# TongtongSong/OpenEAT

Measured on AMD Instinct MI355X. Metric: audio-frames/sec/GPU (train) + RTF (attention-rescoring decode), 12L Conformer, higher is better.
Workload: dtype f32 (storage, accumulate, softmax, norms, losses, optimizer all fp32; every matrix product is the fp32 product to within one fp32 rounding, computed as six exact bf16 x bf16 MFMA products of three-piece operand splits h+m+l = x, dropped terms < 2^-24 |a||b| - tests hold it to the exact-fp32 mode's t; 1 GPU; configs[1]: 12L Conformer d=256 (12+3+3, h=4, ff=1024, K=15, V=3246), B=32/GPU x 10 s 16 kHz wav (T=998 frames), L=30, CTC+attention joint loss, fbank+fwd+bwd+clip+Adam, dropout 0.1; global_batch=32, parallelism=dp1, hip_graph=True

## Files before the change

openeat_amd/csrc/conv.hip:

```cpp
#include <stdlib.h>
#include "oe_common.h"
#include "../../include/openeat_hip.h"

__global__ __launch_bounds__(256) void conv1_fwd_kernel(const float* __restrict__ x, const float* __restrict__ w,
                                                         const float* __restrict__ bias, int B, int T, int F, int T1, int F1,
                                                         int C, int pos_per_block, float* __restrict__ y,
                                                         __bf16* __restrict__ y_planes, long plane_stride) {
    const int cpt = C >> 2;
    const int grp = threadIdx.x / cpt;
    const int c4 = (threadIdx.x % cpt) * 4;
    const int ngrp = blockDim.x / cpt;
    float wr[4][9], br[4];
#pragma unroll
    for (int e = 0; e < 4; ++e) {
        br[e] = bias[c4 + e];
#pragma unroll
        for (int k = 0; k < 9; ++k) wr[e][k] = w[(c4 + e) * 9 + k];
    }
    const long npos = (long)B * T1 * F1;
    const long p0 = (long)blockIdx.x * pos_per_block;
    for (long pos = p0 + grp; pos < min(npos, p0 + pos_per_block); pos += ngrp) {
        const int f = (int)(pos % F1);
        const int t = (int)((pos / F1) % T1);
        const long b = pos / ((long)F1 * T1);
        const float* xp = x + (b * T + 2 * t) * F + 2 * f;
        float xv[9];
#pragma unroll
        for (int kh = 0; kh < 3; ++kh)
#pragma unroll
            for (int kw = 0; kw < 3; ++kw) xv[kh * 3 + kw] = xp[kh * F + kw];
        float o[4];
#pragma unroll
        for (int e = 0; e < 4; ++e) {
            float s = br[e];
#pragma unroll
            for (int k = 0; k < 9; ++k) s += wr[e][k] * xv[k];
            o[e] = fmaxf(s, 0.f);
        }
        const float4 o4 = make_float4(o[0], o[1], o[2], o[3]);
        if (y) *reinterpret_cast<float4*>(y + pos * C + c4) = o4;
        if (y_planes) store_planes4(y_planes + pos * C + c4, plane_stride, o4);
    }
}

template <int UB, bool UNIFORM>
__global__ __launch_bounds__(UNIFORM ? 512 : 256) void conv1_wgrad_kernel(const float* __restrict__ x, const float* __restrict__ dy, int B, int T,
                                                           int F, int T1, int F1, int C, int pos_per_block,
                                                           float* __restrict__ dw, float* __restrict__ db) {
    const int cpt = C >> 2;
    const int grp = UNIFORM ? __builtin_amdgcn_readfirstlane(threadIdx.x >> 6) : threadIdx.x / cpt;
    const int c4 = (threadIdx.x % cpt) * 4;
    const int ngrp = blockDim.x / cpt;
    float acc[4][10];
#pragma unroll
    for (int e = 0; e < 4; ++e)
#pragma unroll
        for (int k = 0; k < 10; ++k) acc[e][k] = 0.f;
    const long npos = (long)B * T1 * F1;
    const long p0 = (long)blockIdx.x * pos_per_block;
    const long pstart = p0 + grp, pend = min(npos, p0 + pos_per_block);
    int f = (int)(pstart % F1), t = (int)((pstart / F1) % T1);
    long b = pstart / ((long)F1 * T1);
    for (long pos = pstart; pos < pend; pos += (long)UB * ngrp) {
        float xv[UB][9];
        float4 g4[UB];
#pragma unroll
        for (int u = 0; u < UB; ++u) {
            const long pu = pos + (long)u * ngrp;
            const bool ok = pu < pend;
            const float* xp = x + (b * T + 2 * t) * F + 2 * f;
#pragma unroll
            for (int kh = 0; kh < 3; ++kh)
#pragma unroll
                for (int kw = 0; kw < 3; ++kw) xv[u][kh * 3 + kw] = ok ? xp[kh * F + kw] : 0.f;
            g4[u] = ok ? *reinterpret_cast<const float4*>(dy + pu * C + c4) : make_float4(0.f, 0.f, 0.f, 0.f);
            f += ngrp;
            while (f >= F1) { f -= F1; if (++t == T1) { t = 0; ++b; } }
            if (b >= B) { b = B - 1; t = 0; f = 0; }
        }
#pragma unroll
        for (int u = 0; u < UB; ++u) {
            const float g[4] = {g4[u].x, g4[u].y, g4[u].z, g4[u].w};
#pragma unroll
            for (int e = 0; e < 4; ++e) {
#pragma unroll
                for (int k = 0; k < 9; ++k) acc[e][k] += g[e] * xv[u][k];
                acc[e][9] += g[e];
            }
        }
    }
    extern __shared__ float sh[];
    if (UNIFORM) {
        for (int i = threadIdx.x; i < C * 10; i += blockDim.x) sh[i] = 0.f;
        __syncthreads();
#pragma unroll
        for (int e = 0; e < 4; ++e)
#pragma unroll
            for (int k = 0; k < 10; ++k) atomicAdd(&sh[(c4 + e) * 10 + k], acc[e][k]);
        __syncthreads();
        for (int i = threadIdx.x; i < C * 10; i += blockDim.x) {
            const int c = i / 10, k = i % 10;
            if (k < 9) atomicAdd(dw + c * 9 + k, sh[i]); else atomicAdd(db + c, sh[i]);
        }
        return;
    }
#pragma unroll
    for (int e = 0; e < 4; ++e)
#pragma unroll
        for (int k = 0; k < 10; ++k) sh[(grp * C + c4 + e) * 10 + k] = acc[e][k];
    __syncthreads();
    for (int i = threadIdx.x; i < C * 10; i += blockDim.x) {
        float s = 0.f;
        for (int gq = 0; gq < ngrp; ++gq) s += sh[gq * C * 10 + i];
        const int c = i / 10, k = i % 10;
        if (k < 9) atomicAdd(dw + c * 9 + k, s); else atomicAdd(db + c, s);
    }
}

static int conv1_block(int C) {
    const int cpt = C / 4;
    return cpt * (256 / cpt > 0 ? 256 / cpt : 1);
}

extern "C" int oe_conv1_fwd_pl(const float* x, const float* w, const float* bias, int B, int T, int F, int C, float* y,
                               void* y_planes, long plane_stride, void* stream);
extern "C" int oe_conv1_fwd(const float* x, const float* w, const float* bias, int B, int T, int F, int C, float* y,
                            void* stream) {
    return oe_conv1_fwd_pl(x, w, bias, B, T, F, C, y, nullptr, 0, stream);
}
extern "C" int oe_conv1_fwd_pl(const float* x, const float* w, const float* bias, int B, int T, int F, int C, float* y,
                               void* y_planes, long plane_stride, void* stream) {
    OE_REQUIRE(x && w && bias && (y || y_planes), "oe_conv1_fwd: null pointer");
    OE_REQUIRE(!y_planes || ((((uintptr_t)y_planes) & 7) == 0 && plane_stride % 4 == 0), "oe_conv1_fwd_pl: planes must be 8-byte aligned");
    OE_REQUIRE(B > 0 && T >= 3 && F >= 3 && C > 0 && C % 4 == 0 && C <= 1024, "oe_conv1_fwd: bad shape (C %% 4 == 0, C <= 1024)");
    const int T1 = (T - 3) / 2 + 1, F1 = (F - 3) / 2 + 1;
    const long npos = (long)B * T1 * F1;
    const int ppb = 64;
    hipLaunchKernelGGL(conv1_fwd_kernel, dim3(oe_cdiv(npos, ppb)), dim3(conv1_block(C)), 0, (hipStream_t)stream, x, w, bias, B, T,
                       F, T1, F1, C, ppb, y, (__bf16*)y_planes, plane_stride);
    OE_LAUNCH_CHECK("conv1_fwd");
    return 0;
}

extern "C" int oe_conv1_wgrad(const float* x, const float* dy, int B, int T, int F, int C, float* dw, float* db, void* stream) {
    OE_REQUIRE(x && dy && dw && db, "oe_conv1_wgrad: null pointer");
    OE_REQUIRE(B > 0 && T >= 3 && F >= 3 && C > 0 && C % 4 == 0 && C <= 1024, "oe_conv1_wgrad: bad shape");
    const int T1 = (T - 3) / 2 + 1, F1 = (F - 3) / 2 + 1;
    const long npos = (long)B * T1 * F1;
    static const int ppb_env = getenv("OE_CONV1_WGRAD_PPB") ? atoi(getenv("OE_CONV1_WGRAD_PPB")) : 0;
    static const int variant = getenv("OE_CONV1_WGRAD") ? atoi(getenv("OE_CONV1_WGRAD")) : 0;
    const bool uni = (C == 256) && variant != 1;
    const int ppb = ppb_env > 0 ? ppb_env : (uni ? (int)max(256L, (npos + 511) / 512) : 512);
    const int threads = uni ? 512 : conv1_block(C);
    const int ngrp = threads / (C / 4);
    const size_t lds = uni ? (size_t)C * 10 * sizeof(float) : (size_t)ngrp * C * 10 * sizeof(float);
#define C1W(UBB, UNI) hipLaunchKernelGGL((conv1_wgrad_kernel<UBB, UNI>), dim3(oe_cdiv(npos, ppb)), dim3(threads), lds, (hipStream_t)stream, x, dy, B, T, F, T1,  \
                                         F1, C, ppb, dw, db)
    if (uni && variant == 8) C1W(8, true);
    else if (uni) C1W(4, true);
    else if (variant == 1) C1W(1, false);
    else C1W(4, false);
#undef C1W
    OE_LAUNCH_CHECK("conv1_wgrad");
    return 0;
}

__global__ __launch_bounds__(256) void col2im_relu_kernel(const float* __restrict__ dcol, const float* __restrict__ y1, int B,
                                                           int T1, int F1, int T2, int F2, int C, int KS, int S,
                                                           float* __restrict__ dx) {
    const long idx = (long)blockIdx.x * blockDim.x + threadIdx.x;
    const int cv = C >> 2;
    const long total = (long)B * T1 * F1 * cv;
    if (idx >= total) return;
    const int c = (int)(idx % cv) * 4;
    const long pos = idx / cv;
    const int f1 = (int)(pos % F1);
    const int t1 = (int)((pos / F1) % T1);
    const long b = pos / ((long)F1 * T1);
    float4 s = make_float4(0.f, 0.f, 0.f, 0.f);
    for (int kh = 0; kh < KS; ++kh) {
        const int tt = t1 - kh;
        if (tt < 0 || (tt % S) || (tt / S) >= T2) continue;
        for (int kw = 0; kw < KS; ++kw) {
            const int ff = f1 - kw;
            if (ff < 0 || (ff % S) || (ff / S) >= F2) continue;
            const long m = (b * T2 + (tt / S)) * F2 + (ff / S);
            const float4 v = *reinterpret_cast<const float4*>(dcol + m * ((long)KS * KS * C) + (kh * KS + kw) * C + c);
            s.x += v.x; s.y += v.y; s.z += v.z; s.w += v.w;
        }
    }
    const float4 y = *reinterpret_cast<const float4*>(y1 + pos * C + c);
    s.x = y.x > 0.f ? s.x : 0.f; s.y = y.y > 0.f ? s.y : 0.f; s.z = y.z > 0.f ? s.z : 0.f; s.w = y.w > 0.f ? s.w : 0.f;
    *reinterpret_cast<float4*>(dx + pos * C + c) = s;
}

extern "C" int oe_col2im_relu_ks(const float* dcol, const float* y1, int B, int T1, int F1, int C, int KS, int S, float* dx,
                                 void* stream) {
    OE_REQUIRE(dcol && y1 && dx && B > 0 && KS >= 1 && S >= 1 && T1 >= KS && F1 >= KS && C > 0 && C % 4 == 0, "oe_col2im_relu: bad arguments");
    const int T2 = (T1 - KS) / S + 1, F2 = (F1 - KS) / S + 1;
    const long total = (long)B * T1 * F1 * (C / 4);
    hipLaunchKernelGGL(col2im_relu_kernel, dim3(oe_cdiv(total, 256)), dim3(256), 0, (hipStream_t)stream, dcol, y1, B, T1, F1, T2,
                       F2, C, KS, S, dx);
    OE_LAUNCH_CHECK("col2im_relu");
    return 0;
}
extern "C" int oe_col2im_relu(const float* dcol, const float* y1, int B, int T1, int F1, int C, float* dx, void* stream) {
    return oe_col2im_relu_ks(dcol, y1, B, T1, F1, C, 3, 2, dx, stream);
}

#ifdef OE_GEMM_STAMPS
static __device__ unsigned long long* oe_dw_stamp_buf = nullptr;
extern "C" int oe_debug_set_dw_stamp_buffer(void* p) { return (int)hipMemcpyToSymbol(HIP_SYMBOL(oe_dw_stamp_buf), &p, sizeof(p)); }
#define DW_STAMP(slot)                                                                                         \
    do {                                                                                                       \
        __builtin_amdgcn_sched_barrier(0);                                                                     \
        unsigned long long t_;                                                                                 \
        asm volatile("s_memtime %0\n\ts_waitcnt lgkmcnt(0)" : "=s"(t_) :: "memory");                           \
        __builtin_amdgcn_sched_barrier(0);                                                                     \
        if (oe_dw_stamp_buf && threadIdx.x == 0 && blockIdx.y < 8) oe_dw_stamp_buf[(blockIdx.y * 16 + (blockIdx.x & 15)) * 8 + (slot)] = t_; \
    } while (0)
#else
#define DW_STAMP(slot) do { } while (0)
#endif

#define DW_TT 16
#define DW_MAXK 31
template <int KT, bool EXACT>
__global__ __launch_bounds__(256) void dwconv_glu_fwd_kernel(const float* __restrict__ a, const float* __restrict__ w,
                                                              const float* __restrict__ bias, const float* __restrict__ gpad,
                                                              int T, int d, int K, int pad_left, float* __restrict__ y,
                                                              const float* __restrict__ ln_gamma, const float* __restrict__ ln_beta, float ln_eps,
                                                              int ln_act, float* __restrict__ z, float* __restrict__ ln_stats) {
    extern __shared__ __attribute__((aligned(16))) float win[];
    const int b = blockIdx.y;
    const int t0 = blockIdx.x * DW_TT;
    const int rows = DW_TT + K - 1;
    const int dv = d >> 2;
    for (int e0 = threadIdx.x; e0 < rows * dv; e0 += 256 * 4) {
        float4 xv[4], gv[4];
        int kind[4];
#pragma unroll
        for (int u = 0; u < 4; ++u) {
            const int e = e0 + u * 256;
            kind[u] = 0;
            xv[u] = gv[u] = make_float4(0.f, 0.f, 0.f, 0.f);
            if (e < rows * dv) {
                const int r = e / dv, c = (e % dv) * 4;
                const int t = t0 - pad_left + r;
                if (t >= 0 && t < T) {
                    const float* ap = a + ((long)b * T + t) * 2 * d;
                    xv[u] = *reinterpret_cast<const float4*>(ap + c);
                    gv[u] = *reinterpret_cast<const float4*>(ap + d + c);
                    kind[u] = 1;
                } else if (t < 0 && gpad) {
                    xv[u] = *reinterpret_cast<const float4*>(gpad + c);
                    kind[u] = 2;
                }
            }
        }
#pragma unroll
        for (int u = 0; u < 4; ++u) {
            const int e = e0 + u * 256;
            if (e < rows * dv) {
                const int r = e / dv, c = (e % dv) * 4;
                float4 g = xv[u];
                if (kind[u] == 1)
                    g = make_float4(xv[u].x * sigmoidf_(gv[u].x), xv[u].y * sigmoidf_(gv[u].y), xv[u].z * sigmoidf_(gv[u].z), xv[u].w * sigmoidf_(gv[u].w));
                *reinterpret_cast<float4*>(win + r * d + c) = g;
            }
        }
    }
    __syncthreads();
    for (int c = threadIdx.x; c < d; c += 256) {
        float wk[KT];
#pragma unroll
        for (int k = 0; k < KT; ++k) wk[k] = (EXACT || k < K) ? w[c * K + k] : 0.f;
        const float bc = bias[c];
#pragma unroll
        for (int tt = 0; tt < DW_TT; ++tt) {
            const int t = t0 + tt;
            float s = bc;
#pragma unroll
            for (int k = 0; k < KT; ++k) if (EXACT || k < K) s += wk[k] * win[(tt + k) * d + c];
            if (t < T) y[((long)b * T + t) * d + c] = s;
            if (z) win[(rows + tt) * d + c] = s;
        }
    }
    if (z == nullptr) return;
    __syncthreads();
    const int lane = threadIdx.x & 63, wave = threadIdx.x >> 6;
    const float4* g4 = reinterpret_cast<const float4*>(ln_gamma);
    const float4* b4 = reinterpret_cast<const float4*>(ln_beta);
    for (int tt = wave; tt < DW_TT; tt += 4) {
        const int t = t0 + tt;
        if (t >= T) break;
        const float4* yr = reinterpret_cast<const float4*>(win + (rows + tt) * d);
        float sum = 0.f;
        for (int i = lane; i < dv; i += 64) { const float4 v = yr[i]; sum += v.x + v.y + v.z + v.w; }
        const float mean = wave_sum(sum) / d;
        float q = 0.f;
        for (int i = lane; i < dv; i += 64) {
            const float4 v = yr[i];
            const float p0 = v.x - mean, p1 = v.y - mean, p2 = v.z - mean, p3 = v.w - mean;
            q += p0 * p0 + p1 * p1 + p2 * p2 + p3 * p3;
        }
        const float rstd = rsqrtf(wave_sum(q) / d + ln_eps);
        const long row = (long)b * T + t;
        if (lane == 0) { ln_stats[row * 2] = mean; ln_stats[row * 2 + 1] = rstd; }
        float4* zr = reinterpret_cast<float4*>(z + row * d);
        for (int i = lane; i < dv; i += 64) {
            const float4 v = yr[i], g = g4[i], bb = b4[i];
            zr[i] = make_float4(act_fwd(ln_act, (v.x - mean) * rstd * g.x + bb.x), act_fwd(ln_act, (v.y - mean) * rstd * g.y + bb.y),
                                act_fwd(ln_act, (v.z - mean) * rstd * g.z + bb.z), act_fwd(ln_act, (v.w - mean) * rstd * g.w + bb.w));
        }
    }
}

template <int KT, bool EXACT>
__global__ __launch_bounds__(256) void dwconv_glu_bwd_kernel(const float* __restrict__ a, const float* __restrict__ dy,
                                                              const float* __restrict__ w, const float* __restrict__ gpad,
                                                              int T, int d, int K, int pad_left,
                                                              float* __restrict__ da, float* __restrict__ partial,
                                                              float* __restrict__ dgpad) {
    extern __shared__ __attribute__((aligned(16))) float sh[];
    const int rows = DW_TT + K - 1;
    float* gwin = sh;
    float* dwin = sh + rows * d;
    const int b = blockIdx.y;
    const int t0 = blockIdx.x * DW_TT;
    const int dv = d >> 2;
    DW_STAMP(0);
    for (int e0 = threadIdx.x; e0 < rows * dv; e0 += 256 * 8) {
        float4 xv[8], gv[8], qv[8];
        int kind[8];
#pragma unroll
        for (int u = 0; u < 8; ++u) {
            const int e = e0 + u * 256;
            kind[u] = 0;
            xv[u] = gv[u] = qv[u] = make_float4(0.f, 0.f, 0.f, 0.f);
            if (e < rows * dv) {
                const int r = e / dv, c = (e % dv) * 4;
                const int tg = t0 - pad_left + r;
                if (tg >= 0 && tg < T) {
                    const float* ap = a + ((long)b * T + tg) * 2 * d;
                    xv[u] = *reinterpret_cast<const float4*>(ap + c);
                    gv[u] = *reinterpret_cast<const float4*>(ap + d + c);
                    kind[u] = 1;
                } else if (tg < 0 && gpad) {
                    xv[u] = *reinterpret_cast<const float4*>(gpad + c);
                    kind[u] = 2;
                }
                const int td = t0 + pad_left - (K - 1) + r;
                if (td >= 0 && td < T) qv[u] = *reinterpret_cast<const float4*>(dy + ((long)b * T + td) * d + c);
            }
        }
#pragma unroll
        for (int u = 0; u < 8; ++u) {
            const int e = e0 + u * 256;
            if (e < rows * dv) {
                const int r = e / dv, c = (e % dv) * 4;
                float4 g = xv[u];
                if (kind[u] == 1)
                    g = make_float4(xv[u].x * sigmoidf_(gv[u].x), xv[u].y * sigmoidf_(gv[u].y), xv[u].z * sigmoidf_(gv[u].z), xv[u].w * sigmoidf_(gv[u].w));
                *reinterpret_cast<float4*>(gwin + r * d + c) = g;
                *reinterpret_cast<float4*>(dwin + r * d + c) = qv[u];
            }
        }
    }
    DW_STAMP(1);
    __syncthreads();
    DW_STAMP(2);
    for (int c = threadIdx.x; c < d; c += 256) {
        float wk[KT], dwk[KT];
#pragma unroll
        for (int k = 0; k < KT; ++k) { wk[k] = (EXACT || k < K) ? w[c * K + k] : 0.f; dwk[k] = 0.f; }
        float dbs = 0.f;
        float xs[DW_TT], gs[DW_TT];
#pragma unroll
        for (int tt = 0; tt < DW_TT; ++tt) {
            const int t = min(t0 + tt, T - 1);
            const float* ap = a + ((long)b * T + t) * 2 * d;
            xs[tt] = ap[c];
            gs[tt] = ap[d + c];
        }
        DW_STAMP(3);
#pragma unroll
        for (int tt = 0; tt < DW_TT; ++tt) {
            const int t = t0 + tt;
            if (t < T) {
            float dg = 0.f;
#pragma unroll
            for (int k = 0; k < KT; ++k) if (EXACT || k < K) dg += wk[k] * dwin[(tt + (K - 1) - k) * d + c];
            const float xv = xs[tt], gv = gs[tt];
            const float sg = sigmoidf_(gv);
            float* dap = da + ((long)b * T + t) * 2 * d;
            dap[c] = dg * sg;
            dap[d + c] = dg * xv * sg * (1.f - sg);
            const float dyt = dwin[(tt + (K - 1) - pad_left) * d + c];
            dbs += dyt;
#pragma unroll
            for (int k = 0; k < KT; ++k) if (EXACT || k < K) dwk[k] += dyt * gwin[(tt + k) * d + c];
            }
        }
        DW_STAMP(4);
        float* pp = partial + ((long)(blockIdx.y * gridDim.x + blockIdx.x) * (K + 1)) * d + c;
#pragma unroll
        for (int k = 0; k < KT; ++k) if (EXACT || k < K) pp[(long)k * d] = dwk[k];
        pp[(long)K * d] = dbs;
        DW_STAMP(5);
        if (dgpad && blockIdx.x == 0) {
            float acc = 0.f;
            const int td0 = pad_left - (K - 1);
            for (int tau = -pad_left; tau < 0; ++tau)
#pragma unroll
                for (int k = 0; k < KT; ++k) {
                    const int td = tau + pad_left - k;
                    if ((EXACT || k < K) && td >= 0 && td - td0 < rows) acc += wk[k] * dwin[(td - td0) * d + c];
                }
            atomicAdd(dgpad + c, acc);
        }
    }
}

#define DW_PR_ROWS 64
__global__ __launch_bounds__(256) void dwconv_param_reduce_kernel(const float* __restrict__ partial, int nblocks, int d, int K,
                                                                   float* __restrict__ dw, float* __restrict__ db) {
    __shared__ float sh[4][64];
    const int cx = threadIdx.x & 63, ry = threadIdx.x >> 6;
    const int idx = blockIdx.x * 64 + cx;
    const int n = (K + 1) * d;
    const int b0 = blockIdx.y * DW_PR_ROWS, b1 = min(nblocks, b0 + DW_PR_ROWS);
    float s = 0.f;
    if (idx < n) {
#pragma unroll 4
        for (int b = b0 + ry; b < b1; b += 4) s += partial[(long)b * n + idx];
    }
    sh[ry][cx] = s;
    __syncthreads();
    if (ry == 0 && idx < n) {
        const float v = sh[0][cx] + sh[1][cx] + sh[2][cx] + sh[3][cx];
        const int k = idx / d, c = idx % d;
        if (k < K) atomicAdd(dw + c * K + k, v); else atomicAdd(db + c, v);
    }
}

extern "C" size_t oe_dwconv_glu_bwd_workspace_floats(int B, int T, int d, int K) {
    return (size_t)B * oe_cdiv(T, DW_TT) * (K + 1) * d;
}

extern "C" int oe_dwconv_glu_ln_fwd(const float* a, const float* w, const float* bias, const float* gpad, int B, int T, int d,
                                    int K, int causal, float* y, const float* ln_gamma, const float* ln_beta, float ln_eps, int ln_act,
                                    float* z, float* ln_stats, void* stream);
extern "C" int oe_dwconv_glu_fwd(const float* a, const float* w, const float* bias, const float* gpad, int B, int T, int d,
                                 int K, int causal, float* y, void* stream) {
    return oe_dwconv_glu_ln_fwd(a, w, bias, gpad, B, T, d, K, causal, y, nullptr, nullptr, 0.f, 0, nullptr, nullptr, stream);
}
extern "C" int oe_dwconv_glu_ln_fwd(const float* a, const float* w, const float* bias, const float* gpad, int B, int T, int d,
                                    int K, int causal, float* y, const float* ln_gamma, const float* ln_beta, float ln_eps, int ln_act,
                                    float* z, float* ln_stats, void* stream) {
    OE_REQUIRE(a && w && bias && y, "oe_dwconv_glu_fwd: null pointer");
    OE_REQUIRE(!z || (ln_gamma && ln_beta && ln_stats), "oe_dwconv_glu_ln_fwd: the fused LayerNorm needs gamma, beta and a statistics buffer");
    OE_REQUIRE(B > 0 && T > 0 && d > 0 && d % 4 == 0 && K >= 1 && K <= DW_MAXK, "oe_dwconv_glu_fwd: bad shape (d %% 4, K <= %d)", DW_MAXK);
    OE_REQUIRE(causal || (K % 2 == 1), "oe_dwconv_glu_fwd: kernel size must be odd for the symmetric convolution");
    const int pad_left = causal ? K - 1 : (K - 1) / 2;
    const size_t lds = (size_t)(DW_TT + K - 1 + (z ? DW_TT : 0)) * d * sizeof(float);
    OE_REQUIRE(lds <= 160 * 1024, "oe_dwconv_glu_fwd: window does not fit LDS (d=%d)", d);
#define DW_FWD(KT, EX)                                                                                                           \
    do {                                                                                                                     \
        if (lds > 48 * 1024) (void)hipFuncSetAttribute((const void*)dwconv_glu_fwd_kernel<KT, EX>, hipFuncAttributeMaxDynamicSharedMemorySize, (int)lds); \
        hipLaunchKernelGGL((dwconv_glu_fwd_kernel<KT, EX>), dim3(oe_cdiv(T, DW_TT), B), dim3(256), lds, (hipStream_t)stream, a, w, bias, gpad, T, d, \
                           K, pad_left, y, ln_gamma, ln_beta, ln_eps, ln_act, z, ln_stats);                                  \
    } while (0)
    if (K == 15) DW_FWD(15, true); else if (K == 7) DW_FWD(7, true); else if (K == 31) DW_FWD(31, true);
    else if (K < 7) DW_FWD(7, false); else if (K < 15) DW_FWD(15, false); else DW_FWD(31, false);
#undef DW_FWD
    OE_LAUNCH_CHECK("dwconv_glu_fwd");
    return 0;
}

extern "C" int oe_dwconv_glu_bwd(const float* a, const float* dy, const float* w, const float* gpad, int B, int T, int d, int K,
                                 int causal, float* da, float* dw, float* db, float* dgpad, float* workspace, void* stream) {
    OE_REQUIRE(a && dy && w && da && dw && db && workspace, "oe_dwconv_glu_bwd: null pointer");
    OE_REQUIRE(!dgpad || (K - 1 <= DW_TT + K - 1), "oe_dwconv_glu_bwd: pad window");
    OE_REQUIRE(B > 0 && T > 0 && d > 0 && d % 4 == 0 && K >= 1 && K <= DW_MAXK, "oe_dwconv_glu_bwd: bad shape");
    const int pad_left = causal ? K - 1 : (K - 1) / 2;
    const size_t lds = (size_t)2 * (DW_TT + K - 1) * d * sizeof(float);
    OE_REQUIRE(lds <= 160 * 1024, "oe_dwconv_glu_bwd: window does not fit LDS (d=%d)", d);
#define DW_BWD(KT, EX)                                                                                                           \
    do {                                                                                                                     \
        if (lds > 48 * 1024) (void)hipFuncSetAttribute((const void*)dwconv_glu_bwd_kernel<KT, EX>, hipFuncAttributeMaxDynamicSharedMemorySize, (int)lds); \
        hipLaunchKernelGGL((dwconv_glu_bwd_kernel<KT, EX>), dim3(oe_cdiv(T, DW_TT), B), dim3(256), lds, (hipStream_t)stream, a, dy, w, gpad, T, d, \
                           K, pad_left, da, workspace, dgpad);                                                               \
    } while (0)
    if (K == 15) DW_BWD(15, true); else if (K == 7) DW_BWD(7, true); else if (K == 31) DW_BWD(31, true);
    else if (K < 7) DW_BWD(7, false); else if (K < 15) DW_BWD(15, false); else DW_BWD(31, false);
#undef DW_BWD
    OE_LAUNCH_CHECK("dwconv_glu_bwd");
    hipLaunchKernelGGL(dwconv_param_reduce_kernel, dim3(oe_cdiv((K + 1) * d, 64), oe_cdiv(B * oe_cdiv(T, DW_TT), DW_PR_ROWS)), dim3(256), 0, (hipStream_t)stream, workspace,
                       B * oe_cdiv(T, DW_TT), d, K, dw, db);
    OE_LAUNCH_CHECK("dwconv_param_reduce");
    return 0;
}


__global__ __launch_bounds__(256) void pad1_nhwc_kernel(const float4* __restrict__ dy, int B, int To, int Fo, int C4, float4* __restrict__ out) {
    const long n = (long)B * (To + 2) * (Fo + 2) * C4;
    for (long i = (long)blockIdx.x * 256 + threadIdx.x; i < n; i += (long)gridDim.x * 256) {
        const int c = (int)(i % C4);
        long q = i / C4;
        const int f = (int)(q % (Fo + 2)) - 1;
        q /= (Fo + 2);
        const int t = (int)(q % (To + 2)) - 1;
        const long b = q / (To + 2);
        float4 v = make_float4(0.f, 0.f, 0.f, 0.f);
        if (t >= 0 && t < To && f >= 0 && f < Fo) v = dy[((b * To + t) * Fo + f) * C4 + c];
        out[i] = v;
    }
}
extern "C" int oe_pad1_nhwc(const float* dy, int B, int To, int Fo, int C, float* out, void* stream) {
    OE_REQUIRE(dy && out && B > 0 && To > 0 && Fo > 0 && C > 0 && C % 4 == 0, "oe_pad1_nhwc: bad arguments (C must be a multiple of 4)");
    OE_REQUIRE((((uintptr_t)dy | (uintptr_t)out) & 15) == 0, "oe_pad1_nhwc: pointers must be 16-byte aligned");
    const long n = (long)B * (To + 2) * (Fo + 2) * (C / 4);
    hipLaunchKernelGGL(pad1_nhwc_kernel, dim3((unsigned)min((long)oe_cdiv(n, 256), 65536L)), dim3(256), 0, (hipStream_t)stream,
                       (const float4*)dy, B, To, Fo, C / 4, (float4*)out);
    OE_LAUNCH_CHECK("pad1_nhwc");
    return 0;
}
__global__ __launch_bounds__(256) void pad1_nhwc_planes_kernel(const float4* __restrict__ dy, int B, int To, int Fo, int C4, float4* __restrict__ out,
                                                                __bf16* __restrict__ planes, long pstride) {
    const long n = (long)B * (To + 2) * (Fo + 2) * C4;
    for (long i = (long)blockIdx.x * 256 + threadIdx.x; i < n; i += (long)gridDim.x * 256) {
        const int c = (int)(i % C4);
        long q = i / C4;
        const int f = (int)(q % (Fo + 2)) - 1;
        q /= (Fo + 2);
        const int t = (int)(q % (To + 2)) - 1;
        const long b = q / (To + 2);
        float4 v = make_float4(0.f, 0.f, 0.f, 0.f);
        if (t >= 0 && t < To && f >= 0 && f < Fo) v = dy[((b * To + t) * Fo + f) * C4 + c];
        if (out) out[i] = v;
        store_planes4(planes + 4 * i, pstride, v);
    }
}
extern "C" int oe_pad1_nhwc_planes(const float* dy, int B, int To, int Fo, int C, float* out, void* planes, long plane_stride, void* stream) {
    OE_REQUIRE(dy && planes && B > 0 && To > 0 && Fo > 0 && C > 0 && C % 4 == 0, "oe_pad1_nhwc_planes: bad arguments (C must be a multiple of 4)");
    OE_REQUIRE((((uintptr_t)dy | (uintptr_t)out) & 15) == 0 && (((uintptr_t)planes) & 7) == 0 && plane_stride % 4 == 0,
               "oe_pad1_nhwc_planes: dy / out must be 16-byte, the planes 8-byte aligned");
    const long n = (long)B * (To + 2) * (Fo + 2) * (C / 4);
    hipLaunchKernelGGL(pad1_nhwc_planes_kernel, dim3((unsigned)min((long)oe_cdiv(n, 256), 65536L)), dim3(256), 0, (hipStream_t)stream,
                       (const float4*)dy, B, To, Fo, C / 4, (float4*)out, (__bf16*)planes, plane_stride);
    OE_LAUNCH_CHECK("pad1_nhwc_planes");
    return 0;
}
__global__ __launch_bounds__(256) void conv_dgrad_k3s2_weights_kernel(const float* __restrict__ w, int C, float* __restrict__ out) {
    const long n = 9L * C * C;
    const long i = (long)blockIdx.x * 256 + threadIdx.x;
    if (i >= n) return;
    const long cc = (long)C * C;
    int cls, KH, KW;
    long base;
    if (i < 4 * cc) { cls = 0; KH = 2; KW = 2; base = 0; }
    else if (i < 6 * cc) { cls = 1; KH = 2; KW = 1; base = 4 * cc; }
    else if (i < 8 * cc) { cls = 2; KH = 1; KW = 2; base = 6 * cc; }
    else { cls = 3; KH = 1; KW = 1; base = 8 * cc; }
    const long r = i - base;
    const int co = (int)(r % C);
    long q = r / C;
    const int kwi = (int)(q % KW);
    q /= KW;
    const int khi = (int)(q % KH);
    const int ci = (int)(q / KH);
    const int kh = (cls >> 1) ? 1 : (khi == 0 ? 2 : 0);
    const int kw = (cls & 1) ? 1 : (kwi == 0 ? 2 : 0);
    out[i] = w[(((long)co * C + ci) * 3 + kh) * 3 + kw];
}
extern "C" int oe_conv_dgrad_k3s2_weights(const float* w, int C, float* out, void* stream) {
    OE_REQUIRE(w && out && C > 0, "oe_conv_dgrad_k3s2_weights: bad arguments");
    hipLaunchKernelGGL(conv_dgrad_k3s2_weights_kernel, dim3(oe_cdiv(9L * C * C, 256)), dim3(256), 0, (hipStream_t)stream, w, C, out);
    OE_LAUNCH_CHECK("conv_dgrad_k3s2_weights");
    return 0;
}
```

openeat_amd/csrc/fbank.hip:

```cpp
#include "oe_common.h"
#include "../../include/openeat_hip.h"

#define FB_WAVES 4
#define FB_MAX_NFFT 1024

#define FB_WAVE_SYNC()                                            \
    do {                                                          \
        asm volatile("s_waitcnt lgkmcnt(0)" ::: "memory");        \
        __builtin_amdgcn_wave_barrier();                          \
    } while (0)
template <int FB_NFFT>
__global__ __launch_bounds__(64 * FB_WAVES) void fbank_kernel(const float* __restrict__ wav, const int* __restrict__ nsamples,
                                                              int B, long wav_stride, int Tmax, int win, int hop, int n_mel,
                                                              float scale, float preemph, const float* __restrict__ window,
                                                              const float* __restrict__ twiddle, const int* __restrict__ mel_start,
                                                              const int* __restrict__ mel_off, const float* __restrict__ mel_w,
                                                              float floor_eps, const float* __restrict__ cmvn_mean,
                                                              const float* __restrict__ cmvn_istd, float* __restrict__ out,
                                                              float dither, unsigned long long dither_seed) {
    __shared__ float2 bufA[FB_WAVES][FB_NFFT];
    __shared__ float2 bufB[FB_WAVES][FB_NFFT];
    __shared__ float2 tw[FB_NFFT / 2];
    for (int i = threadIdx.x; i < FB_NFFT / 2; i += 64 * FB_WAVES) tw[i] = reinterpret_cast<const float2*>(twiddle)[i];
    __syncthreads();
    const int lane = threadIdx.x & 63, wave = threadIdx.x >> 6;
    const long frame = (long)blockIdx.x * FB_WAVES + wave;
    const bool live_frame = frame < (long)B * Tmax;
    const int b = live_frame ? (int)(frame / Tmax) : 0;
    const int t = live_frame ? (int)(frame % Tmax) : 0;
    const int ns = nsamples ? nsamples[b] : (int)wav_stride;
    const int Tb = ns < win ? 0 : 1 + (ns - win) / hop;
    const bool live = live_frame && t < Tb;
    float2* A = bufA[wave];
    float2* Bf = bufB[wave];
    float part = 0.f;
    const float* src = wav + (long)b * wav_stride + (long)t * hop;
    for (int i = lane; i < FB_NFFT; i += 64) {
        float v = 0.f;
        if (live && i < win) {
            v = src[i] * scale;
            if (dither != 0.f) {
                const uint4 h = philox4(dither_seed, (unsigned long long)frame * FB_NFFT + i);
                const float u1 = ((float)(h.x >> 8) + 0.5f) * (1.f / 16777216.f), u2 = (float)(h.y >> 8) * (1.f / 16777216.f);
                v += dither * sqrtf(-2.f * __logf(u1)) * __cosf(6.283185307179586f * u2);
            }
        }
        A[i].x = v;
        part += v;
    }
    const float mean = wave_sum(part) / (float)win;
    FB_WAVE_SYNC();
    for (int i = lane; i < FB_NFFT; i += 64) {
        float v = 0.f;
        if (i < win) {
            const float cur = A[i].x - mean;
            const float prev = A[i > 0 ? i - 1 : 0].x - mean;
            v = (cur - preemph * prev) * window[i];
        }
        Bf[i] = make_float2(v, 0.f);
    }
    FB_WAVE_SYNC();
    float2* s0 = Bf;
    float2* s1 = A;
#pragma unroll 1
    for (int Ns = 1; Ns < FB_NFFT; Ns <<= 1) {
        for (int j = lane; j < FB_NFFT / 2; j += 64) {
            const int k = j & (Ns - 1);
            const float2 w = tw[k * (FB_NFFT / 2 / Ns)];
            const float2 u = s0[j];
            const float2 x1 = s0[j + FB_NFFT / 2];
            const float2 v = make_float2(x1.x * w.x - x1.y * w.y, x1.x * w.y + x1.y * w.x);
            const int base = ((j - k) << 1) + k;
            s1[base] = make_float2(u.x + v.x, u.y + v.y);
            s1[base + Ns] = make_float2(u.x - v.x, u.y - v.y);
        }
        FB_WAVE_SYNC();
        float2* tmp = s0; s0 = s1; s1 = tmp;
    }
    for (int i = lane; i <= FB_NFFT / 2; i += 64) {
        const float2 c = s0[i];
        s1[i].x = c.x * c.x + c.y * c.y;
    }
    FB_WAVE_SYNC();
    if (!live_frame) return;
    float* dst = out + ((long)b * Tmax + t) * n_mel;
    for (int m = lane; m < n_mel; m += 64) {
        float r = 0.f;
        if (live) {
            const int st = mel_start[m], o0 = mel_off[m], o1 = mel_off[m + 1];
            float acc = 0.f;
            for (int q = o0; q < o1; ++q) acc += mel_w[q] * s1[st + (q - o0)].x;
            r = __logf(fmaxf(acc, floor_eps));
            if (cmvn_mean) r = (r - cmvn_mean[m]) * cmvn_istd[m];
        }
        dst[m] = r;
    }
}

extern "C" int oe_fbank(const float* wav, const int* nsamples, int B, long wav_stride, int Tmax, int win, int hop, int n_mel,
                        float scale, float preemph, const float* window, const float* twiddle, const int* mel_start,
                        const int* mel_off, const float* mel_w, float floor_eps, const float* cmvn_mean,
                        const float* cmvn_istd, float* out, void* stream) {
    return oe_fbank_dither(wav, nsamples, B, wav_stride, Tmax, win, hop, n_mel, scale, preemph, window, twiddle, mel_start, mel_off,
                           mel_w, floor_eps, cmvn_mean, cmvn_istd, 0.f, 0ull, out, stream);
}

extern "C" int oe_fbank_dither(const float* wav, const int* nsamples, int B, long wav_stride, int Tmax, int win, int hop, int n_mel,
                               float scale, float preemph, const float* window, const float* twiddle, const int* mel_start,
                               const int* mel_off, const float* mel_w, float floor_eps, const float* cmvn_mean,
                               const float* cmvn_istd, float dither, unsigned long long seed, float* out, void* stream) {
    OE_REQUIRE(wav && window && twiddle && mel_start && mel_off && mel_w && out, "oe_fbank: null pointer");
    OE_REQUIRE(B > 0 && Tmax > 0 && win > 0 && win <= FB_MAX_NFFT && hop > 0 && n_mel > 0, "oe_fbank: bad shape (window must be <= %d samples)", FB_MAX_NFFT);
    OE_REQUIRE(nsamples || wav_stride >= (long)(Tmax - 1) * hop + win, "oe_fbank: Tmax frames do not fit in wav_stride samples");
    OE_REQUIRE((cmvn_mean == nullptr) == (cmvn_istd == nullptr), "oe_fbank: cmvn mean/istd must come together");
    const long frames = (long)B * Tmax;
#define FB_LAUNCH(NF) hipLaunchKernelGGL(fbank_kernel<NF>, dim3(oe_cdiv(frames, FB_WAVES)), dim3(64 * FB_WAVES), 0, (hipStream_t)stream, wav, nsamples, \
                       B, wav_stride, Tmax, win, hop, n_mel, scale, preemph, window, twiddle, mel_start, mel_off, mel_w, floor_eps,                  \
                       cmvn_mean, cmvn_istd, out, dither, seed)
    if (win <= 128) FB_LAUNCH(128); else if (win <= 256) FB_LAUNCH(256); else if (win <= 512) FB_LAUNCH(512); else FB_LAUNCH(1024);
#undef FB_LAUNCH
    OE_LAUNCH_CHECK("fbank");
    return 0;
}

#define UN_RG 16
__global__ __launch_bounds__(1024) void utt_norm_kernel(float* __restrict__ x, const int* __restrict__ nframes, int Tmax, int F) {
    __shared__ float sh[2][UN_RG][64];
    const int b = blockIdx.x;
    const int cx = threadIdx.x & 63;
    const int f = blockIdx.y * 64 + cx;
    const int ry = threadIdx.x >> 6;
    const int Tb = nframes ? min(nframes[b], Tmax) : Tmax;
    float* base = x + (long)b * Tmax * F + (f < F ? f : 0);
    const bool on = f < F;
    float s0 = 0.f, s1 = 0.f, s2 = 0.f, s3 = 0.f;
    int t = ry;
    if (on) {
        for (; t + 3 * UN_RG < Tb; t += 4 * UN_RG) {
            s0 += base[(long)t * F]; s1 += base[(long)(t + UN_RG) * F]; s2 += base[(long)(t + 2 * UN_RG) * F]; s3 += base[(long)(t + 3 * UN_RG) * F];
        }
        for (; t < Tb; t += UN_RG) s0 += base[(long)t * F];
    }
    sh[0][ry][cx] = (s0 + s1) + (s2 + s3);
    __syncthreads();
    float m = 0.f;
#pragma unroll
    for (int r = 0; r < UN_RG; ++r) m += sh[0][r][cx];
    const float mean = m / (float)max(Tb, 1);
    float q0 = 0.f, q1 = 0.f, q2 = 0.f, q3 = 0.f;
    if (on) {
        for (t = ry; t + 3 * UN_RG < Tb; t += 4 * UN_RG) {
            const float d0 = base[(long)t * F] - mean, d1 = base[(long)(t + UN_RG) * F] - mean;
            const float d2 = base[(long)(t + 2 * UN_RG) * F] - mean, d3 = base[(long)(t + 3 * UN_RG) * F] - mean;
            q0 += d0 * d0; q1 += d1 * d1; q2 += d2 * d2; q3 += d3 * d3;
        }
        for (; t < Tb; t += UN_RG) { const float d = base[(long)t * F] - mean; q0 += d * d; }
    }
    sh[1][ry][cx] = (q0 + q1) + (q2 + q3);
    __syncthreads();
    float v = 0.f;
#pragma unroll
    for (int r = 0; r < UN_RG; ++r) v += sh[1][r][cx];
    const float inv = 1.f / sqrtf(v / (float)max(Tb, 1));
    if (on) {
        for (t = ry; t + 3 * UN_RG < Tb; t += 4 * UN_RG) {
            const float a0 = base[(long)t * F], a1 = base[(long)(t + UN_RG) * F], a2 = base[(long)(t + 2 * UN_RG) * F], a3 = base[(long)(t + 3 * UN_RG) * F];
            base[(long)t * F] = (a0 - mean) * inv; base[(long)(t + UN_RG) * F] = (a1 - mean) * inv;
            base[(long)(t + 2 * UN_RG) * F] = (a2 - mean) * inv; base[(long)(t + 3 * UN_RG) * F] = (a3 - mean) * inv;
        }
        for (; t < Tb; t += UN_RG) base[(long)t * F] = (base[(long)t * F] - mean) * inv;
    }
}

extern "C" int oe_utt_normalize(float* x, const int* nframes, int B, int Tmax, int F, void* stream) {
    OE_REQUIRE(x && B > 0 && Tmax > 0 && F > 0, "oe_utt_normalize: bad arguments");
    hipLaunchKernelGGL(utt_norm_kernel, dim3(B, oe_cdiv(F, 64)), dim3(64 * UN_RG), 0, (hipStream_t)stream, x, nframes, Tmax, F);
    OE_LAUNCH_CHECK("utt_normalize");
    return 0;
}
```

Baseline: 2.007 million audio-frames/s.

## Rework fbank FFT as packed real radix-4 and widen/pipeline conv1 kernels

The fbank kernel now packs the real frame into a half-length complex FFT. It runs radix-4 stages with a final radix-2 where needed, then unpacks to the power spectrum. This cuts LDS traffic, the number of sync stages and the buffer size, and lets padded frames exit early after writing zeros. The conv1 forward kernel gains an 8-channel-per-thread path with wave-uniform position groups and incremental index updates instead of per-position div/mod. The conv1 weight-grad kernel double-buffers the dy loads with sched barriers to overlap memory and FMA work. These are several independent changes across two kernels; the FFT rewrite risks small rounding differences and the padding path must stay correct.

```diff
diff --git a/openeat_amd/csrc/conv.hip b/openeat_amd/csrc/conv.hip
--- a/openeat_amd/csrc/conv.hip
+++ b/openeat_amd/csrc/conv.hip
@@ -2,47 +2,81 @@
 #include "oe_common.h"
 #include "../../include/openeat_hip.h"
 
+template <int CH, int PW>
 __global__ __launch_bounds__(256) void conv1_fwd_kernel(const float* __restrict__ x, const float* __restrict__ w,
                                                          const float* __restrict__ bias, int B, int T, int F, int T1, int F1,
                                                          int C, int pos_per_block, float* __restrict__ y,
                                                          __bf16* __restrict__ y_planes, long plane_stride) {
-    const int cpt = C >> 2;
-    const int grp = threadIdx.x / cpt;
-    const int c4 = (threadIdx.x % cpt) * 4;
+    const int cpt = C / CH;
+    const int grp = PW > 0 ? __builtin_amdgcn_readfirstlane(threadIdx.x / cpt) : threadIdx.x / cpt;
+    const int sub = PW == 2 ? (threadIdx.x >> 5) & 1 : 0;
+    const int c0 = (threadIdx.x % cpt) * CH;
     const int ngrp = blockDim.x / cpt;
-    float wr[4][9], br[4];
-#pragma unroll
-    for (int e = 0; e < 4; ++e) {
-        br[e] = bias[c4 + e];
-#pragma unroll
-        for (int k = 0; k < 9; ++k) wr[e][k] = w[(c4 + e) * 9 + k];
+    float wr[CH][9], br[CH];
+#pragma unroll
+    for (int e = 0; e < CH; ++e) {
+        br[e] = bias[c0 + e];
+#pragma unroll
+        for (int k = 0; k < 9; ++k) wr[e][k] = w[(c0 + e) * 9 + k];
     }
     const long npos = (long)B * T1 * F1;
     const long p0 = (long)blockIdx.x * pos_per_block;
-    for (long pos = p0 + grp; pos < min(npos, p0 + pos_per_block); pos += ngrp) {
-        const int f = (int)(pos % F1);
-        const int t = (int)((pos / F1) % T1);
-        const long b = pos / ((long)F1 * T1);
-        const float* xp = x + (b * T + 2 * t) * F + 2 * f;
+    const long pstart = p0 + grp, pend = min(npos, p0 + pos_per_block);
+    if (pstart >= pend) return;
+    int b = (int)(pstart / ((long)F1 * T1));
+    const int rem = (int)(pstart - (long)b * F1 * T1);
+    int t = rem / F1, f = rem % F1;
+    for (long pg = pstart; pg < pend; pg += ngrp) {
+        const float* xp = x + ((long)b * T + 2 * t) * F + 2 * f;
         float xv[9];
 #pragma unroll
         for (int kh = 0; kh < 3; ++kh)
 #pragma unroll
             for (int kw = 0; kw < 3; ++kw) xv[kh * 3 + kw] = xp[kh * F + kw];
-        float o[4];
-#pragma unroll
-        for (int e = 0; e < 4; ++e) {
+        if (PW == 2) {
+            int f2 = f + 1, t2 = t, b2 = b;
+            if (f2 == F1) { f2 = 0; if (++t2 == T1) { t2 = 0; ++b2; } }
+            if (pg + 1 >= npos) { f2 = f; t2 = t; b2 = b; }
+            const float* xq = x + ((long)b2 * T + 2 * t2) * F + 2 * f2;
+#pragma unroll
+            for (int kh = 0; kh < 3; ++kh)
+#pragma unroll
+                for (int kw = 0; kw < 3; ++kw) {
+                    const float v2 = xq[kh * F + kw];
+                    xv[kh * 3 + kw] = sub ? v2 : xv[kh * 3 + kw];
+                }
+        }
+        f += ngrp;
+        while (f >= F1) { f -= F1; if (++t == T1) { t = 0; ++b; } }
+        const long pos = pg + sub;
+        if (pos >= pend) continue;
+        float o[CH];
+#pragma unroll
+        for (int e = 0; e < CH; ++e) {
             float s = br[e];
 #pragma unroll
             for (int k = 0; k < 9; ++k) s += wr[e][k] * xv[k];
             o[e] = fmaxf(s, 0.f);
         }
-        const float4 o4 = make_float4(o[0], o[1], o[2], o[3]);
-        if (y) *reinterpret_cast<float4*>(y + pos * C + c4) = o4;
-        if (y_planes) store_planes4(y_planes + pos * C + c4, plane_stride, o4);
-    }
-}
-
+        if constexpr (CH == 8) {
+            if (y) {
+                float4* yp = reinterpret_cast<float4*>(y + pos * C + c0);
+                yp[0] = make_float4(o[0], o[1], o[2], o[3]);
+                yp[1] = make_float4(o[4], o[5], o[6], o[7]);
+            }
+            if (y_planes) {
+                oe_bf16x8 pl[3];
+                oe_split8<3>(o, pl);
+#pragma unroll
+                for (int n = 0; n < 3; ++n) *reinterpret_cast<oe_bf16x8*>(y_planes + pos * C + c0 + n * plane_stride) = pl[n];
+            }
+        } else {
+            const float4 o4 = make_float4(o[0], o[1], o[2], o[3]);
+            if (y) *reinterpret_cast<float4*>(y + pos * C + c0) = o4;
+            if (y_planes) store_planes4(y_planes + pos * C + c0, plane_stride, o4);
+        }
+    }
+}
 template <int UB, bool UNIFORM>
 __global__ __launch_bounds__(UNIFORM ? 512 : 256) void conv1_wgrad_kernel(const float* __restrict__ x, const float* __restrict__ dy, int B, int T,
                                                            int F, int T1, int F1, int C, int pos_per_block,
@@ -59,34 +93,59 @@
     const long npos = (long)B * T1 * F1;
     const long p0 = (long)blockIdx.x * pos_per_block;
     const long pstart = p0 + grp, pend = min(npos, p0 + pos_per_block);
-    int f = (int)(pstart % F1), t = (int)((pstart / F1) % T1);
-    long b = pstart / ((long)F1 * T1);
-    for (long pos = pstart; pos < pend; pos += (long)UB * ngrp) {
-        float xv[UB][9];
-        float4 g4[UB];
+    int b = (int)(pstart / ((long)F1 * T1));
+    const int rem = (int)(pstart - (long)b * F1 * T1);
+    int t = rem / F1, f = rem % F1;
+    if (b >= B) { b = B - 1; t = 0; f = 0; }
+    const int rend = (int)(pend - p0);
+    const int step = UB * ngrp;
+    const float* dyb = dy + p0 * C + c4;
+    constexpr int TB = UB < 4 ? UB : 4;
+    auto issue = [&](int r, float4 (&g)[UB]) {
 #pragma unroll
         for (int u = 0; u < UB; ++u) {
-            const long pu = pos + (long)u * ngrp;
-            const bool ok = pu < pend;
-            const float* xp = x + (b * T + 2 * t) * F + 2 * f;
+            const int ru = min(r + u * ngrp, rend - 1);
+            g[u] = *reinterpret_cast<const float4*>(dyb + (size_t)ru * C);
+        }
+    };
+    auto taps = [&](float (&xv)[TB][9]) {
+#pragma unroll
+        for (int u = 0; u < TB; ++u) {
+            const float* xp = x + ((long)b * T + 2 * t) * F + 2 * f;
 #pragma unroll
             for (int kh = 0; kh < 3; ++kh)
 #pragma unroll
-                for (int kw = 0; kw < 3; ++kw) xv[u][kh * 3 + kw] = ok ? xp[kh * F + kw] : 0.f;
-            g4[u] = ok ? *reinterpret_cast<const float4*>(dy + pu * C + c4) : make_float4(0.f, 0.f, 0.f, 0.f);
+                for (int kw = 0; kw < 3; ++kw) xv[u][kh * 3 + kw] = xp[kh * F + kw];
             f += ngrp;
             while (f >= F1) { f -= F1; if (++t == T1) { t = 0; ++b; } }
             if (b >= B) { b = B - 1; t = 0; f = 0; }
         }
+    };
+    auto group = [&](int r, const float4 (&g)[UB], float4 (&gnext)[UB]) {
+        float xv[TB][9];
+        taps(xv);
+        issue(r + step, gnext);
+        __builtin_amdgcn_sched_barrier(0);
 #pragma unroll
         for (int u = 0; u < UB; ++u) {
-            const float g[4] = {g4[u].x, g4[u].y, g4[u].z, g4[u].w};
+            if (u > 0 && u % TB == 0) taps(xv);
+            const bool ok = r + u * ngrp < rend;
+            const float gv[4] = {ok ? g[u].x : 0.f, ok ? g[u].y : 0.f, ok ? g[u].z : 0.f, ok ? g[u].w : 0.f};
 #pragma unroll
             for (int e = 0; e < 4; ++e) {
 #pragma unroll
-                for (int k = 0; k < 9; ++k) acc[e][k] += g[e] * xv[u][k];
-                acc[e][9] += g[e];
-            }
+                for (int k = 0; k < 9; ++k) acc[e][k] += gv[e] * (ok ? xv[u % TB][k] : 0.f);
+                acc[e][9] += gv[e];
+            }
+        }
+        __builtin_amdgcn_sched_barrier(0);
+    };
+    if (grp < rend) {
+        float4 g0[UB], g1[UB];
+        issue(grp, g0);
+        for (int r = grp; r < rend; r += 2 * step) {
+            group(r, g0, g1);
+            group(r + step, g1, g0);
         }
     }
     extern __shared__ float sh[];
@@ -135,9 +194,18 @@
     OE_REQUIRE(B > 0 && T >= 3 && F >= 3 && C > 0 && C % 4 == 0 && C <= 1024, "oe_conv1_fwd: bad shape (C %% 4 == 0, C <= 1024)");
     const int T1 = (T - 3) / 2 + 1, F1 = (F - 3) / 2 + 1;
     const long npos = (long)B * T1 * F1;
-    const int ppb = 64;
-    hipLaunchKernelGGL(conv1_fwd_kernel, dim3(oe_cdiv(npos, ppb)), dim3(conv1_block(C)), 0, (hipStream_t)stream, x, w, bias, B, T,
-                       F, T1, F1, C, ppb, y, (__bf16*)y_planes, plane_stride);
+    static const int ppb_env = getenv("OE_CONV1_FWD_PPB") ? atoi(getenv("OE_CONV1_FWD_PPB")) : 0;
+    const int ppb = ppb_env > 0 ? ppb_env : 64;
+    const bool wide = C % 8 == 0 && (((uintptr_t)y) & 15) == 0 && (((uintptr_t)y_planes) & 15) == 0 && plane_stride % 8 == 0;
+    const int cpt = C / (wide ? 8 : 4);
+    const int threads = cpt * (256 / cpt > 0 ? 256 / cpt : 1);
+#define C1F(CH, PW) hipLaunchKernelGGL((conv1_fwd_kernel<CH, PW>), dim3(oe_cdiv(npos, ppb)), dim3(threads), 0, (hipStream_t)stream, x, w, bias, B, T,  \
+                                       F, T1, F1, C, ppb, y, (__bf16*)y_planes, plane_stride)
+    if (wide && cpt % 64 == 0) C1F(8, 1);
+    else if (wide && cpt == 32) C1F(8, 2);
+    else if (wide) C1F(8, 0);
+    else C1F(4, 0);
+#undef C1F
     OE_LAUNCH_CHECK("conv1_fwd");
     return 0;
 }
@@ -150,7 +218,7 @@
     static const int ppb_env = getenv("OE_CONV1_WGRAD_PPB") ? atoi(getenv("OE_CONV1_WGRAD_PPB")) : 0;
     static const int variant = getenv("OE_CONV1_WGRAD") ? atoi(getenv("OE_CONV1_WGRAD")) : 0;
     const bool uni = (C == 256) && variant != 1;
-    const int ppb = ppb_env > 0 ? ppb_env : (uni ? (int)max(256L, (npos + 511) / 512) : 512);
+    const int ppb = ppb_env > 0 ? min(ppb_env, 1 << 24) : (uni ? (int)min(1L << 24, max(256L, (npos + 511) / 512)) : 512);
     const int threads = uni ? 512 : conv1_block(C);
     const int ngrp = threads / (C / 4);
     const size_t lds = uni ? (size_t)C * 10 * sizeof(float) : (size_t)ngrp * C * 10 * sizeof(float);
diff --git a/openeat_amd/csrc/fbank.hip b/openeat_amd/csrc/fbank.hip
--- a/openeat_amd/csrc/fbank.hip
+++ b/openeat_amd/csrc/fbank.hip
@@ -9,6 +9,54 @@
         asm volatile("s_waitcnt lgkmcnt(0)" ::: "memory");        \
         __builtin_amdgcn_wave_barrier();                          \
     } while (0)
+
+__device__ __forceinline__ float2 fb_cmul(float2 a, float2 w) { return make_float2(a.x * w.x - a.y * w.y, a.x * w.y + a.y * w.x); }
+template <int NFFT>
+__device__ __forceinline__ float2 fb_tw(const float2* tw, int idx) {
+    const float2 w = tw[idx & (NFFT / 2 - 1)];
+    return idx >= NFFT / 2 ? make_float2(-w.x, -w.y) : w;
+}
+__device__ __forceinline__ void fb_radix4(float2 (&v)[4]) {
+    const float2 a0 = make_float2(v[0].x + v[2].x, v[0].y + v[2].y), a1 = make_float2(v[0].x - v[2].x, v[0].y - v[2].y);
+    const float2 a2 = make_float2(v[1].x + v[3].x, v[1].y + v[3].y), a3 = make_float2(v[1].y - v[3].y, v[3].x - v[1].x);
+    v[0] = make_float2(a0.x + a2.x, a0.y + a2.y);
+    v[1] = make_float2(a1.x + a3.x, a1.y + a3.y);
+    v[2] = make_float2(a0.x - a2.x, a0.y - a2.y);
+    v[3] = make_float2(a1.x - a3.x, a1.y - a3.y);
+}
+template <int NFFT, int NS>
+__device__ __forceinline__ void fb_stage4(const float2* s0, float2* s1, const float2* tw, int lane) {
+    constexpr int M = NFFT / 2;
+#pragma unroll
+    for (int j0 = 0; j0 < M / 4; j0 += 64) {
+        const int j = j0 + lane;
+        if (M / 4 < 64 && j >= M / 4) break;
+        const int k = j & (NS - 1);
+        float2 v[4];
+#pragma unroll
+        for (int q = 0; q < 4; ++q) v[q] = s0[j + q * (M / 4)];
+#pragma unroll
+        for (int q = 1; q < 4; ++q) v[q] = fb_cmul(v[q], fb_tw<NFFT>(tw, q * k * (M / (2 * NS))));
+        fb_radix4(v);
+        const int base = ((j - k) << 2) + k;
+#pragma unroll
+        for (int q = 0; q < 4; ++q) s1[base + q * NS] = v[q];
+    }
+}
+template <int NFFT>
+__device__ __forceinline__ void fb_stage2(const float2* s0, float2* s1, const float2* tw, int lane) {
+    constexpr int M = NFFT / 2;
+#pragma unroll
+    for (int j0 = 0; j0 < M / 2; j0 += 64) {
+        const int j = j0 + lane;
+        if (M / 2 < 64 && j >= M / 2) break;
+        const float2 u = s0[j];
+        const float2 v = fb_cmul(s0[j + M / 2], tw[2 * j]);
+        s1[j] = make_float2(u.x + v.x, u.y + v.y);
+        s1[j + M / 2] = make_float2(u.x - v.x, u.y - v.y);
+    }
+}
+
 template <int FB_NFFT>
 __global__ __launch_bounds__(64 * FB_WAVES) void fbank_kernel(const float* __restrict__ wav, const int* __restrict__ nsamples,
                                                               int B, long wav_stride, int Tmax, int win, int hop, int n_mel,
@@ -18,81 +66,117 @@
                                                               float floor_eps, const float* __restrict__ cmvn_mean,
                                                               const float* __restrict__ cmvn_istd, float* __restrict__ out,
                                                               float dither, unsigned long long dither_seed) {
-    __shared__ float2 bufA[FB_WAVES][FB_NFFT];
-    __shared__ float2 bufB[FB_WAVES][FB_NFFT];
-    __shared__ float2 tw[FB_NFFT / 2];
-    for (int i = threadIdx.x; i < FB_NFFT / 2; i += 64 * FB_WAVES) tw[i] = reinterpret_cast<const float2*>(twiddle)[i];
+    constexpr int M = FB_NFFT / 2;
+    __shared__ __attribute__((aligned(16))) float2 bufA[FB_WAVES][M];
+    __shared__ __attribute__((aligned(16))) float2 bufB[FB_WAVES][M];
+    __shared__ float2 tw[M];
+    for (int i = threadIdx.x; i < M; i += 64 * FB_WAVES) tw[i] = reinterpret_cast<const float2*>(twiddle)[i];
     __syncthreads();
     const int lane = threadIdx.x & 63, wave = threadIdx.x >> 6;
     const long frame = (long)blockIdx.x * FB_WAVES + wave;
-    const bool live_frame = frame < (long)B * Tmax;
-    const int b = live_frame ? (int)(frame / Tmax) : 0;
-    const int t = live_frame ? (int)(frame % Tmax) : 0;
+    if (frame >= (long)B * Tmax) return;
+    const int b = (int)(frame / Tmax);
+    const int t = (int)(frame % Tmax);
     const int ns = nsamples ? nsamples[b] : (int)wav_stride;
     const int Tb = ns < win ? 0 : 1 + (ns - win) / hop;
-    const bool live = live_frame && t < Tb;
+    float* dst = out + ((long)b * Tmax + t) * n_mel;
+    if (t >= Tb) {
+        for (int m = lane; m < n_mel; m += 64) dst[m] = 0.f;
+        return;
+    }
     float2* A = bufA[wave];
     float2* Bf = bufB[wave];
+    float* raw = reinterpret_cast<float*>(A);
+    const float* src = wav + (long)b * wav_stride + (long)t * hop;
+    float sv[FB_NFFT / 64];
+#pragma unroll
+    for (int k = 0; k < FB_NFFT / 64; ++k) sv[k] = src[min(lane + 64 * k, win - 1)];
+    constexpr int NB = (M / 4 + 63) / 64;
+    float wv[NB][4][2];
+#pragma unroll
+    for (int jb = 0; jb < NB; ++jb)
+#pragma unroll
+        for (int q = 0; q < 4; ++q) {
+            const int n = min(jb * 64 + lane, M / 4 - 1) + q * (M / 4);
+            wv[jb][q][0] = window[min(2 * n, win - 1)];
+            wv[jb][q][1] = window[min(2 * n + 1, win - 1)];
+        }
     float part = 0.f;
-    const float* src = wav + (long)b * wav_stride + (long)t * hop;
-    for (int i = lane; i < FB_NFFT; i += 64) {
-        float v = 0.f;
-        if (live && i < win) {
-            v = src[i] * scale;
-            if (dither != 0.f) {
-                const uint4 h = philox4(dither_seed, (unsigned long long)frame * FB_NFFT + i);
-                const float u1 = ((float)(h.x >> 8) + 0.5f) * (1.f / 16777216.f), u2 = (float)(h.y >> 8) * (1.f / 16777216.f);
-                v += dither * sqrtf(-2.f * __logf(u1)) * __cosf(6.283185307179586f * u2);
-            }
-        }
-        A[i].x = v;
+#pragma unroll
+    for (int k = 0; k < FB_NFFT / 64; ++k) {
+        const int i = lane + 64 * k;
+        float v = sv[k] * scale;
+        if (dither != 0.f) {
+            const uint4 h = philox4(dither_seed, (unsigned long long)frame * FB_NFFT + i);
+            const float u1 = ((float)(h.x >> 8) + 0.5f) * (1.f / 16777216.f), u2 = (float)(h.y >> 8) * (1.f / 16777216.f);
+            v += dither * sqrtf(-2.f * __logf(u1)) * __cosf(6.283185307179586f * u2);
+        }
+        v = i < win ? v : 0.f;
+        raw[i] = v;
         part += v;
     }
     const float mean = wave_sum(part) / (float)win;
     FB_WAVE_SYNC();
-    for (int i = lane; i < FB_NFFT; i += 64) {
-        float v = 0.f;
-        if (i < win) {
-            const float cur = A[i].x - mean;
-            const float prev = A[i > 0 ? i - 1 : 0].x - mean;
-            v = (cur - preemph * prev) * window[i];
-        }
-        Bf[i] = make_float2(v, 0.f);
-    }
-    FB_WAVE_SYNC();
-    float2* s0 = Bf;
-    float2* s1 = A;
-#pragma unroll 1
-    for (int Ns = 1; Ns < FB_NFFT; Ns <<= 1) {
-        for (int j = lane; j < FB_NFFT / 2; j += 64) {
-            const int k = j & (Ns - 1);
-            const float2 w = tw[k * (FB_NFFT / 2 / Ns)];
-            const float2 u = s0[j];
-            const float2 x1 = s0[j + FB_NFFT / 2];
-            const float2 v = make_float2(x1.x * w.x - x1.y * w.y, x1.x * w.y + x1.y * w.x);
-            const int base = ((j - k) << 1) + k;
-            s1[base] = make_float2(u.x + v.x, u.y + v.y);
-            s1[base + Ns] = make_float2(u.x - v.x, u.y - v.y);
-        }
+    auto windowed = [&](int i, float wc) {
+        const float cur = raw[i] - mean;
+        const float prev = raw[i > 0 ? i - 1 : 0] - mean;
+        const float v = (cur - preemph * prev) * wc;
+        return i < win ? v : 0.f;
+    };
+#pragma unroll
+    for (int j0 = 0; j0 < M / 4; j0 += 64) {
+        const int j = j0 + lane;
+        if (M / 4 < 64 && j >= M / 4) break;
+        float2 v[4];
+#pragma unroll
+        for (int q = 0; q < 4; ++q) {
+            const int n = j + q * (M / 4);
+            v[q] = make_float2(windowed(2 * n, wv[j0 / 64][q][0]), windowed(2 * n + 1, wv[j0 / 64][q][1]));
+        }
+        fb_radix4(v);
+        float4* o = reinterpret_cast<float4*>(Bf + 4 * j);
+        o[0] = make_float4(v[0].x, v[0].y, v[1].x, v[1].y);
+        o[1] = make_float4(v[2].x, v[2].y, v[3].x, v[3].y);
+    }
+    FB_WAVE_SYNC();
+    fb_stage4<FB_NFFT, 4>(Bf, A, tw, lane);
+    FB_WAVE_SYNC();
+    fb_stage4<FB_NFFT, 16>(A, Bf, tw, lane);
+    FB_WAVE_SYNC();
+    const float2* Z = Bf;
+    float* pw = reinterpret_cast<float*>(A);
+    if constexpr (M == 128) {
+        fb_stage2<FB_NFFT>(Bf, A, tw, lane);
         FB_WAVE_SYNC();
-        float2* tmp = s0; s0 = s1; s1 = tmp;
-    }
-    for (int i = lane; i <= FB_NFFT / 2; i += 64) {
-        const float2 c = s0[i];
-        s1[i].x = c.x * c.x + c.y * c.y;
-    }
-    FB_WAVE_SYNC();
-    if (!live_frame) return;
-    float* dst = out + ((long)b * Tmax + t) * n_mel;
+        Z = A; pw = reinterpret_cast<float*>(Bf);
+    } else if constexpr (M >= 256) {
+        fb_stage4<FB_NFFT, 64>(Bf, A, tw, lane);
+        FB_WAVE_SYNC();
+        Z = A; pw = reinterpret_cast<float*>(Bf);
+        if constexpr (M == 512) {
+            fb_stage2<FB_NFFT>(A, Bf, tw, lane);
+            FB_WAVE_SYNC();
+            Z = Bf; pw = reinterpret_cast<float*>(A);
+        }
+    }
+#pragma unroll
+    for (int k0 = 0; k0 < M; k0 += 64) {
+        const int k = k0 + lane;
+        const float2 zk = Z[k], zm = Z[(M - k) & (M - 1)];
+        const float2 e = make_float2(0.5f * (zk.x + zm.x), 0.5f * (zk.y - zm.y));
+        const float2 o = make_float2(0.5f * (zk.y + zm.y), 0.5f * (zm.x - zk.x));
+        const float2 wo = fb_cmul(o, tw[k]);
+        const float xr = e.x + wo.x, xi = e.y + wo.y;
+        pw[k] = xr * xr + xi * xi;
+        if (k == 0) { const float ny = zk.x - zk.y; pw[M] = ny * ny; }
+    }
+    FB_WAVE_SYNC();
     for (int m = lane; m < n_mel; m += 64) {
-        float r = 0.f;
-        if (live) {
-            const int st = mel_start[m], o0 = mel_off[m], o1 = mel_off[m + 1];
-            float acc = 0.f;
-            for (int q = o0; q < o1; ++q) acc += mel_w[q] * s1[st + (q - o0)].x;
-            r = __logf(fmaxf(acc, floor_eps));
-            if (cmvn_mean) r = (r - cmvn_mean[m]) * cmvn_istd[m];
-        }
+        const int st = mel_start[m], o0 = mel_off[m], o1 = mel_off[m + 1];
+        float acc = 0.f;
+        for (int q = o0; q < o1; ++q) acc += mel_w[q] * pw[st + (q - o0)];
+        float r = __logf(fmaxf(acc, floor_eps));
+        if (cmvn_mean) r = (r - cmvn_mean[m]) * cmvn_istd[m];
         dst[m] = r;
     }
 }
```

Result: no change. 2.024 million audio-frames/s, median of 6 (+0.9%).
